# kendricktan/simple-zk-rollups

Measured on AMD Instinct MI355X. Metric: Groth16 proofs/sec (rollup batch circuit), higher is better.
Workload: dtype u32 limbs, 254-bit integer Montgomery (9 x 29 bits in the MSM kernels, 8 x 32 bits elsewhere); 1 GPU; 2^20-constraint synthetic rollup circuit, 1 proof per step per GPU; log_m=20, n_public=73, nVars=1048576, nnzA=1827887, nnzB=1577678, parallelism=proof-sharded x1 (key arena replicated once: single), proofs_in_flight=2

## Files before the change

### simple-zk-rollups_amd/csrc/curve29.hpp

```cpp
#pragma once
#include "curve.hpp"
#include "field29.hpp"

namespace zkr {

struct G1C {
  template <int H> using T = L29<Fq29, H>;
  using W = Fq;
  template <int H> static ZKR_HD T<H> unpack(const Fq &w) { return unpack29<Fq29, H>(w.v); }
  template <int H> static ZKR_HD Fq pack(const T<H> &a) { Fq r; pack29(a, r.v); return r; }
  static ZKR_HD T<2> one() { return one29<Fq29>(); }
  static ZKR_HD T<2> to256() { return const29<Fq29>(Fq29::TO256); }
  static ZKR_HD T<2> to261() { return const29<Fq29>(Fq29::TO261); }
};
struct G2C {
  template <int H> using T = Q29<H>;
  using W = Fq2;
  template <int H> static ZKR_HD T<H> unpack(const Fq2 &w) { return Q29<H>{unpack29<Fq29, H>(w.a.v), unpack29<Fq29, H>(w.b.v)}; }
  template <int H> static ZKR_HD Fq2 pack(const T<H> &x) { Fq2 r; pack29(x.a, r.a.v); pack29(x.b, r.b.v); return r; }
  static ZKR_HD T<2> one() { return Q29<2>{one29<Fq29>(), L29<Fq29, 2>::zero()}; }
  static ZKR_HD T<2> to256() { return Q29<2>{const29<Fq29>(Fq29::TO256), L29<Fq29, 2>::zero()}; }
  static ZKR_HD T<2> to261() { return Q29<2>{const29<Fq29>(Fq29::TO261), L29<Fq29, 2>::zero()}; }
};
template <class F> struct CoordOf;
template <> struct CoordOf<Fq> { using C = G1C; };
template <> struct CoordOf<Fq2> { using C = G2C; };

constexpr int HX = 13, HY = 4;

template <class C>
struct Affine29 {
  typename C::template T<2> x, y;
};
template <class C>
struct XYZZ29 {
  typename C::template T<HX> x;
  typename C::template T<HY> y, zz, zzz;
  static ZKR_HD XYZZ29 inf() {
    XYZZ29 r;
    r.x = decltype(r.x)::zero(); r.y = decltype(r.y)::zero(); r.zz = decltype(r.zz)::zero(); r.zzz = decltype(r.zzz)::zero();
    return r;
  }
  ZKR_HD bool is_inf() const { return zz.all_zero(); }
};
template <class C, class X, class Y, class ZZ, class ZZZ>
ZKR_HD XYZZ29<C> make_xyzz(const X &x, const Y &y, const ZZ &zz, const ZZZ &zzz) {
  XYZZ29<C> r;
  r.x = x.template to<HX>(); r.y = y.template to<HY>(); r.zz = zz.template to<HY>(); r.zzz = zzz.template to<HY>();
  return r;
}

template <class F>
ZKR_HD Affine29<typename CoordOf<F>::C> unpack_affine(const Affine<F> &p) {
  using C = typename CoordOf<F>::C;
  return Affine29<C>{C::template unpack<2>(p.x), C::template unpack<2>(p.y)};
}
template <class F>
ZKR_HD XYZZ29<typename CoordOf<F>::C> unpack_xyzz(const XYZZ<F> &p) {
  using C = typename CoordOf<F>::C;
  XYZZ29<C> r;
  r.x = C::template unpack<HY>(p.x).template to<HX>();
  r.y = C::template unpack<HY>(p.y); r.zz = C::template unpack<HY>(p.zz); r.zzz = C::template unpack<HY>(p.zzz);
  return r;
}
template <class F>
ZKR_HD XYZZ<F> pack_xyzz(const XYZZ29<typename CoordOf<F>::C> &p) {
  using C = typename CoordOf<F>::C;
  if (p.is_inf()) return XYZZ<F>::inf();
  return XYZZ<F>{C::template pack<3>(weak(p.x)), C::template pack<HY>(p.y), C::template pack<HY>(p.zz), C::template pack<HY>(p.zzz)};
}

template <class C, class QX, class QY>
ZKR_HD XYZZ29<C> dbl_affine29(const QX &qx, const QY &qy) {
  auto u = dbl(qy);
  auto v = sqr(u);
  auto w = mul(u, v);
  auto s = mul(qx, v);
  auto xx = sqr(qx);
  auto m = add(dbl(xx), xx);
  auto x3 = sub(sqr(m), dbl(s));
  auto y3 = mul_sub(m, sub_factor(s, x3), w, qy);
  return make_xyzz<C>(x3, y3, v, w);
}

template <class C>
ZKR_HD XYZZ29<C> dbl_xyzz29(const XYZZ29<C> &p) {
  if (p.is_inf()) return p;
  auto u = dbl(p.y);
  auto v = sqr(u);
  auto w = mul(u, v);
  auto s = mul(p.x, v);
  auto xx = sqr(p.x);
  auto m = add(dbl(xx), xx);
  auto x3 = sub(sqr(m), dbl(s));
  auto y3 = mul_sub(m, sub_factor(s, x3), w, p.y);
  return make_xyzz<C>(x3, y3, mul(v, p.zz), mul(w, p.zzz));
}

#if defined(__HIP_DEVICE_COMPILE__)
#define ZKR_PIN_ORDER() __builtin_amdgcn_sched_barrier(0)
#else
#define ZKR_PIN_ORDER() ((void)0)
#endif
template <class C>
ZKR_HD XYZZ29<C> add_mixed29(const XYZZ29<C> &acc, const Affine29<C> &q, bool neg_q) {
  if (acc.is_inf()) {
    auto qy = q.y;
    if (neg_q) qy = neg(q.y).template to<2>();
    return make_xyzz<C>(q.x, qy, C::one(), C::one());
  }
  auto u2 = mul(q.x, acc.zz);
  ZKR_PIN_ORDER();
  auto s2 = mul_cneg(q.y, neg_q, acc.zzz);
  ZKR_PIN_ORDER();
  auto p = sub(u2, acc.x);
  auto r = sub(s2, acc.y);
  auto pp = sqr(p);
  if (maybe_zero_mod_p(pp) && is_zero_mod_p(pp)) {
    if (is_zero_mod_p(sqr(r))) {
      auto qy = q.y;
      if (neg_q) qy = neg(q.y).template to<2>();
      return dbl_affine29<C>(q.x, qy);
    }
    return XYZZ29<C>::inf();
  }
  ZKR_PIN_ORDER();
  auto ppp = mul(p, pp);
  ZKR_PIN_ORDER();
  auto qq = mul(acc.x, pp);
  ZKR_PIN_ORDER();
  auto zz3 = mul(acc.zz, pp);
  ZKR_PIN_ORDER();
  auto zzz3 = mul(acc.zzz, ppp);
  ZKR_PIN_ORDER();
  auto x3 = sub_sub_dbl(sqr(r), ppp, qq);
  auto y3 = mul_sub(r, sub_factor(qq, x3), acc.y, ppp);
  return make_xyzz<C>(x3, y3, zz3, zzz3);
}

template <class C, class Again>
ZKR_HD XYZZ29<C> add_full29(const XYZZ29<C> &a, const XYZZ29<C> &b, Again again) {
  if (a.is_inf()) return b;
  if (b.is_inf()) return a;
  auto u1 = mul(a.x, b.zz);
  ZKR_PIN_ORDER();
  auto u2 = mul(b.x, a.zz);
  ZKR_PIN_ORDER();
  auto s1 = mul(a.y, b.zzz);
  ZKR_PIN_ORDER();
  auto s2 = mul(b.y, a.zzz);
  ZKR_PIN_ORDER();
  auto zzp = mul(a.zz, b.zz);
  ZKR_PIN_ORDER();
  auto zzzp = mul(a.zzz, b.zzz);
  ZKR_PIN_ORDER();
  auto p = sub(u2, u1);
  auto r = sub(s2, s1);
  auto pp = sqr(p);
  if (maybe_zero_mod_p(pp) && is_zero_mod_p(pp)) {
    if (is_zero_mod_p(sqr(r))) return dbl_xyzz29(again());
    return XYZZ29<C>::inf();
  }
  ZKR_PIN_ORDER();
  auto ppp = mul(p, pp);
  ZKR_PIN_ORDER();
  auto qq = mul(u1, pp);
  ZKR_PIN_ORDER();
  auto zz3 = mul(zzp, pp);
  ZKR_PIN_ORDER();
  auto zzz3 = mul(zzzp, ppp);
  ZKR_PIN_ORDER();
  auto x3 = sub_sub_dbl(sqr(r), ppp, qq);
  auto y3 = mul_sub(r, sub_factor(qq, x3), s1, ppp);
  return make_xyzz<C>(x3, y3, zz3, zzz3);
}
template <class C>
ZKR_HD XYZZ29<C> add_full29(const XYZZ29<C> &a, const XYZZ29<C> &b) {
  return add_full29<C>(a, b, [&]() { return b; });
}

constexpr int JX = 5, JY = 5, JZ = 8;
template <class C>
struct Jac29 {
  typename C::template T<JX> x;
  typename C::template T<JY> y;
  typename C::template T<JZ> z;
};
template <class C>
ZKR_HD Jac29<C> dbl_jac29(const Jac29<C> &p) {
  auto a = sqr(p.x);
  auto b = sqr(p.y);
  auto c8 = dbl(dbl(dbl(sqr(b))));
  auto s = dbl(dbl(mul(p.x, b)));
  auto e = add(dbl(a), a);
  auto x3 = barrett(sub(sqr(e), dbl(s)));
  auto y3 = barrett(sub(mul(e, sub(s, x3)), c8));
  auto z3 = dbl(mul(p.y, p.z));
  return Jac29<C>{x3.template to<JX>(), y3.template to<JY>(), z3.template to<JZ>()};
}

template <class F>
ZKR_HD_COLD F radix_to_261(const F &w) {
  using C = typename CoordOf<F>::C;
  return C::template pack<2>(canonical(mul(C::template unpack<10>(w), C::to261())));
}
template <class F>
ZKR_HD_COLD F radix_to_256(const F &w) {
  using C = typename CoordOf<F>::C;
  return C::template pack<2>(canonical(mul(C::template unpack<10>(w), C::to256())));
}
template <class F>
ZKR_HD_COLD void radix_to_261_at(F *w) {
  using C = typename CoordOf<F>::C;
  *w = C::template pack<2>(canonical_small(mul(C::template unpack<10>(*w), C::to261())));
}
template <class F>
ZKR_HD_COLD void radix_to_256_at(F *w) {
  using C = typename CoordOf<F>::C;
  *w = C::template pack<2>(canonical_small(mul(C::template unpack<10>(*w), C::to256())));
}
// ... 13 lines not shown
```

### simple-zk-rollups_amd/csrc/field29.hpp

```cpp
#pragma once
#include <utility>
#include "field.hpp"
#include "field29_consts.hpp"

namespace zkr {

constexpr uint32_t M29 = (1u << 29) - 1u;

template <class PM, int H>
struct L29 {
  static_assert(H >= 1 && H <= 128, "value bound out of range: the top limb has to stay below 2^28 (reductions take it as a signed word)");
  static constexpr int bound = H;
  uint32_t v[9];
  static ZKR_HD L29 zero() {
    L29 r;
#pragma unroll
    for (int i = 0; i < 9; i++) r.v[i] = 0;
    return r;
  }
  ZKR_HD bool all_zero() const {
    uint32_t o = 0;
#pragma unroll
    for (int i = 0; i < 9; i++) o |= v[i];
    return o == 0;
// ... 342 lines not shown
  int32_t c = 0;
#pragma unroll
  for (int i = 0; i < 9; i++) {
    t += (uint64_t)q * PM::P[i];
    const uint32_t ti = i < 8 ? (uint32_t)t & M29 : (uint32_t)t;
    t >>= 29;
    const int32_t d = (int32_t)a.v[i] - (int32_t)ti + c;
    if (i < 8) { r.v[i] = (uint32_t)d & M29; c = d >> 29; } else r.v[i] = (uint32_t)d;
  }
  return r;
}
template <class PM, int HA>
ZKR_HD L29<PM, 2> canonical_small(const L29<PM, HA> &a) {
  static_assert(HA <= 6, "reduce first (barrett / weak): one conditional subtraction per half-modulus pair");
  L29<PM, 2> r;
#pragma unroll
  for (int i = 0; i < 9; i++) r.v[i] = a.v[i];
#pragma unroll
  for (int it = 0; it < (HA - 1) / 2; it++) {
    int32_t c = 0;
    uint32_t d[9];
#pragma unroll
    for (int i = 0; i < 9; i++) {
      const int32_t t = (int32_t)r.v[i] - (int32_t)PM::P[i] + c;
      if (i < 8) { d[i] = (uint32_t)t & M29; c = t >> 29; } else { d[i] = (uint32_t)t; c = t >> 31; }
    }
    const bool ge = c == 0;
#pragma unroll
    for (int i = 0; i < 9; i++) r.v[i] = ge ? d[i] : r.v[i];
  }
  return r;
}

template <class PM, int HA>
ZKR_HD bool is_zero_mod_p(const L29<PM, HA> &a) {
  static_assert(HA <= 4, "reduce first: the test compares with 0 and p only");
  uint32_t z = 0, e = 0;
#pragma unroll
  for (int i = 0; i < 9; i++) { z |= a.v[i]; e |= a.v[i] ^ PM::P[i]; }
  return z == 0 || e == 0;
}
template <class PM, int HA>
ZKR_HD bool maybe_zero_mod_p(const L29<PM, HA> &a) {
  static_assert(HA <= 4, "reduce first: the test compares with 0 and p only");
  return a.v[0] == 0 || a.v[0] == PM::P[0];
}
template <class PM, int HA>
ZKR_HD_COLD L29<PM, 2> canonical(const L29<PM, HA> &a) {
  L29<PM, 2> r;
  uint32_t v[9];
#pragma unroll
  for (int i = 0; i < 9; i++) v[i] = a.v[i];
  for (int it = 0; it < (HA + 1) / 2; it++) {
    int32_t c = 0;
    uint32_t d[9];
    for (int i = 0; i < 9; i++) {
      int32_t t = (int32_t)v[i] - (int32_t)PM::P[i] + c;
      if (i < 8) { d[i] = (uint32_t)t & M29; c = t >> 29; } else { d[i] = (uint32_t)t; c = t >> 31; }
    }
    if (c == 0)
      for (int i = 0; i < 9; i++) v[i] = d[i];
  }
#pragma unroll
  for (int i = 0; i < 9; i++) r.v[i] = v[i];
  return r;
}

template <class PM29, class PM, int H = 2>
ZKR_HD L29<PM29, H> limbs_of(const Fp<PM> &a) {
  return unpack29<PM29, H>(a.v);
}
template <class PM, class PM29, int H>
ZKR_HD Fp<PM> words_of(const L29<PM29, H> &a) {
  Fp<PM> r;
  pack29(a, r.v);
  return r;
}

using Fq29 = Fq29Params;
using Fr29 = Fr29Params;

template <int H>
struct Q29 {
  L29<Fq29, H> a, b;
  static ZKR_HD Q29 zero() { return Q29{L29<Fq29, H>::zero(), L29<Fq29, H>::zero()}; }
  ZKR_HD bool all_zero() const { return a.all_zero() && b.all_zero(); }
  template <int H2>
  ZKR_HD Q29<H2> to() const { return Q29<H2>{a.template to<H2>(), b.template to<H2>()}; }
};
constexpr int neg_h(int h) { return 2 * ((h + 1) / 2); }
template <int HA, int HB>
ZKR_HD Q29<HA + HB> add(const Q29<HA> &x, const Q29<HB> &y) { return Q29<HA + HB>{add(x.a, y.a), add(x.b, y.b)}; }
template <int HA>
ZKR_HD Q29<2 * HA> dbl(const Q29<HA> &x) { return Q29<2 * HA>{dbl(x.a), dbl(x.b)}; }
template <int HA, int HB>
ZKR_HD Q29<HA + neg_h(HB)> sub(const Q29<HA> &x, const Q29<HB> &y) { return Q29<HA + neg_h(HB)>{sub(x.a, y.a), sub(x.b, y.b)}; }
template <int HB>
ZKR_HD Q29<neg_h(HB)> neg(const Q29<HB> &y) { return Q29<neg_h(HB)>{neg(y.a), neg(y.b)}; }
template <int HA, int HB, int HC>
ZKR_HD Q29<HA + 2 * ((HB + 2 * HC + 1) / 2)> sub_sub_dbl(const Q29<HA> &x, const Q29<HB> &y, const Q29<HC> &z) {
  return Q29<HA + 2 * ((HB + 2 * HC + 1) / 2)>{sub_sub_dbl(x.a, y.a, z.a), sub_sub_dbl(x.b, y.b, z.b)};
}
constexpr int max_h(int a, int b) { return a > b ? a : b; }
template <int HA, int HB>
ZKR_HD auto mul(const Q29<HA> &x, const Q29<HB> &y) {
  auto re = mul_sum2(x.a, y.a, neg_loose(x.b), y.b);
  auto im = mul_sum2(x.a, y.b, x.b, y.a);
  constexpr int H = max_h(decltype(re)::bound, decltype(im)::bound);
  return Q29<H>{re.template to<H>(), im.template to<H>()};
}
template <int HA>
ZKR_HD auto sqr(const Q29<HA> &x) {
  auto re = mul_sum2(x.a, x.a, neg_loose(x.b), x.b);
  auto im = mul(dbl(x.a), x.b);
  constexpr int H = max_h(decltype(re)::bound, decltype(im)::bound);
  return Q29<H>{re.template to<H>(), im.template to<H>()};
}
template <int HX, int HY, int HZ, int HW>
ZKR_HD auto mul_sub(const Q29<HX> &x, const Q29<HY> &y, const Q29<HZ> &z, const Q29<HW> &w) {
  auto nza = neg_loose(z.a);
  auto re = mul_sum4(x.a, y.a, neg_loose(x.b), y.b, nza, w.a, z.b, w.b);
  auto im = mul_sum4(x.a, y.b, x.b, y.a, nza, w.b, neg_loose(z.b), w.a);
  constexpr int H = max_h(decltype(re)::bound, decltype(im)::bound);
  return Q29<H>{re.template to<H>(), im.template to<H>()};
}
template <int HY, int HZ>
ZKR_HD auto mul_cneg(const Q29<HY> &y, bool flip, const Q29<HZ> &z) {
  auto pa = neg_loose(y.a), pb = neg_loose(y.b), nb = pb;
#pragma unroll
  for (int i = 0; i < 9; i++) {
    const uint32_t na = pa.v[i], nbi = pb.v[i];
    pa.v[i] = flip ? na : y.a.v[i];
    pb.v[i] = flip ? nbi : y.b.v[i];
    nb.v[i] = flip ? y.b.v[i] : nbi;
  }
  auto re = mul_sum2(z.a, pa, z.b, nb);
  auto im = mul_sum2(z.b, pa, z.a, pb);
  constexpr int H = max_h(decltype(re)::bound, decltype(im)::bound);
  return Q29<H>{re.template to<H>(), im.template to<H>()};
}
template <int HA, int HB>
ZKR_HD auto sub_factor(const Q29<HA> &x, const Q29<HB> &y) { return sub(x, y); }
template <int HA>
ZKR_HD Q29<3> weak(const Q29<HA> &x) { return Q29<3>{weak(x.a), weak(x.b)}; }
template <int HA>
ZKR_HD bool is_zero_mod_p(const Q29<HA> &x) { return is_zero_mod_p(x.a) && is_zero_mod_p(x.b); }
template <int HA>
ZKR_HD bool maybe_zero_mod_p(const Q29<HA> &x) { return maybe_zero_mod_p(x.a); }
template <int HA>
ZKR_HD_COLD Q29<2> canonical(const Q29<HA> &x) { return Q29<2>{canonical(x.a), canonical(x.b)}; }

template <int HA>
ZKR_HD Q29<5> barrett(const Q29<HA> &x) { return Q29<5>{barrett(x.a), barrett(x.b)}; }
template <int HA>
ZKR_HD Q29<2> canonical_small(const Q29<HA> &x) { return Q29<2>{canonical_small(x.a), canonical_small(x.b)}; }

template <class PM, int HA>
ZKR_HD L29<PM, 4> inv29(const L29<PM, HA> &a) {
  static_assert(HA * 4 <= 676, "operand bound too wide for the chain's products");
  static_assert(PM::P[0] >= 2, "p - 2 is taken limb-wise without a borrow");
  L29<PM, 4> r = one29<PM>().template to<4>();
#pragma unroll 1
  for (int i = 253; i >= 0; i--) {
    r = sqr(r).template to<4>();
    const uint32_t limb = PM::P[i / 29] - (i / 29 == 0 ? 2u : 0u);
    if ((limb >> (i % 29)) & 1u) r = mul(r, a).template to<4>();
  }
  return r;
}
template <int HA>
ZKR_HD Q29<4> inv29(const Q29<HA> &x) {
  auto ni = inv29(mul_sum2(x.a, x.a, x.b, x.b));
  return Q29<4>{mul(x.a, ni).template to<4>(), mul(neg(x.b), ni).template to<4>()};
}

}
```

### simple-zk-rollups_amd/csrc/host_arith_shim.cpp

```cpp
#include "hostops.hpp"
#include "pairing.hpp"
#include "curve29.hpp"
using namespace zkr;

namespace {
template <class P29> L29<P29, 3> to_m261(const uint8_t *std32) {
  uint32_t w[8];
  memcpy(w, std32, 32);
  return mul(unpack29<P29, 10>(w), const29<P29>(P29::R2)).template to<3>();
}
template <class P29, int H> void from_m261(const L29<P29, H> &x, uint8_t *std32) {
  L29<P29, 2> raw_one = L29<P29, 2>::zero();
  raw_one.v[0] = 1;
  uint32_t w[8];
  pack29(canonical(mul(x, raw_one)), w);
  memcpy(std32, w, 32);
}
template <class P29> void f29_op(int op, const uint8_t *a32, const uint8_t *b32, uint8_t *out) {
  auto a = to_m261<P29>(a32), b = to_m261<P29>(b32);
  switch (op) {
    case 0: from_m261(mul(a, b), out); break;
    case 1: from_m261(sqr(a), out); break;
    case 2: from_m261(add(a, b), out); break;
    case 3: from_m261(sub(a, b), out); break;
    case 4: from_m261(neg(a), out); break;
    case 5: from_m261(mul_sub(a, b, b, a), out); break;
    case 6: from_m261(mul_sum2(a, a, b, b), out); break;
    case 7: {
      auto t = sub(sub(a, b), sub(b, a));
      auto u = add(t, dbl(add(a, b)));
      from_m261(sqr(weak(u)), out);
      break;
    }
    case 8: from_m261(mul_sum4(a, b, a, a, b, b, neg(a), b), out); break;
    case 9: from_m261(weak(sub(sub(sub(a, b), b), b)), out); break;
    case 11: from_m261(mul(a, neg_loose(b)), out); break;
    case 12: from_m261(mul(b, sub_loose(a, b)), out); break;
    case 13: from_m261(mul_sum2(a, sub_loose(a, b), neg_loose(b), a), out); break;
    case 14: from_m261(mul_cneg(a, true, b), out); break;
    case 15: from_m261(mul_cneg(a, false, b), out); break;
    default: from_m261(mul(sub(a, b).template to<17>(), sub(b, a).template to<17>()), out);
  }
}
}

template <class F> static int chain29(const uint8_t *pts, const uint8_t *signs, size_t n, int twice, uint8_t *out) {
  using C = typename CoordOf<F>::C;
  const size_t pb = sizeof(Affine<F>);
  XYZZ29<C> half[2] = {XYZZ29<C>::inf(), XYZZ29<C>::inf()};
  for (size_t i = 0; i < n; i++) {
    Affine<F> p;
    memcpy(&p, pts + i * pb, pb);
    if (p.is_inf()) continue;
    Affine<F> q{radix_to_261(p.x), radix_to_261(p.y)};
    XYZZ29<C> &acc = half[i >= n / 2];
    acc = add_mixed29<C>(acc, unpack_affine(q), signs[i] != 0);
    acc = unpack_xyzz(pack_xyzz<F>(acc));
  }
  XYZZ29<C> tot = add_full29<C>(half[0], half[1]);
  if (twice) tot = add_full29<C>(tot, unpack_xyzz(pack_xyzz<F>(tot)));
  XYZZ<F> res = xyzz_to_256(pack_xyzz<F>(tot));
  if (res.is_inf()) return 1;
  Affine<F> a = to_affine(res);
  if constexpr (sizeof(F) == 32) store_g1_std(out, *reinterpret_cast<G1Affine *>(&a));
  else store_g2_std(out, *reinterpret_cast<G2Affine *>(&a));
  return 0;
}
template <class F> static void jac_levels29(const uint8_t *pt, int c, int levels, uint8_t *out) {
  using C = typename CoordOf<F>::C;
  Affine<F> p;
  memcpy(&p, pt, sizeof p);
  p.x = radix_to_261(p.x); p.y = radix_to_261(p.y);
  Jac29<C> q{C::template unpack<2>(p.x).template to<JX>(), C::template unpack<2>(p.y).template to<JY>(), C::one().template to<JZ>()};
  std::vector<Jac29<C>> lv;
  auto prod = C::one().template to<4>();
  for (int l = 0; l < levels; l++) {
    for (int b = 0; b < c; b++) q = dbl_jac29<C>(q);
    lv.push_back(q);
    prod = mul(prod, q.z).template to<4>();
  }
  auto inv = inv29(prod);
  for (int l = levels - 1; l >= 0; l--) {
    auto pre = C::one().template to<4>();
    for (int j = 0; j < l; j++) pre = mul(pre, lv[j].z).template to<4>();
    auto iz = mul(inv, pre);
    inv = mul(inv, lv[l].z).template to<4>();
    auto iz2 = sqr(iz);
    auto iz3 = mul(iz2, iz);
    Affine<F> a{radix_to_256(C::template pack<2>(canonical_small(mul(lv[l].x, iz2)))), radix_to_256(C::template pack<2>(canonical_small(mul(lv[l].y, iz3))))};
    if constexpr (sizeof(F) == 32) store_g1_std(out + (size_t)l * 64, *reinterpret_cast<G1Affine *>(&a));
    else store_g2_std(out + (size_t)l * 128, *reinterpret_cast<G2Affine *>(&a));
  }
}

#include <atomic>
#include <thread>
#include "shard_group.hpp"

static int shard_group_selftest(unsigned parts, unsigned rounds, unsigned fail_part, unsigned fail_round) {
  zkr::ShardGroup g;
  g.parts = parts;
  g.vecs.resize(parts);
  std::vector<std::atomic<unsigned>> at(parts);
  for (auto &a : at) a.store(0);
  std::atomic<int> bad{0};
  auto work = [&](unsigned i) {
    for (unsigned r = 0; r < rounds; r++) {
      if (i == fail_part && r == fail_round) { g.abort(); return; }
      at[i].store(r + 1);
      const bool ok = g.barrier();
      if (!ok) { if (fail_part >= parts || r < fail_round) bad++; return; }
      for (unsigned j = 0; j < parts; j++)
        if (at[j].load() < r + 1) bad++;
    }
    if (fail_part < parts && fail_round < rounds) bad++;
  };
  std::vector<std::thread> thr;
  for (unsigned i = 1; i < parts; i++) thr.emplace_back(work, i);
  work(0);
  for (auto &t : thr) t.join();
  return bad.load();
}

extern "C" {
int zkr_host_shard_group_selftest(unsigned parts, unsigned rounds, unsigned fail_part, unsigned fail_round) {
  return shard_group_selftest(parts, rounds, fail_part, fail_round);
}
void zkt29_fp(int field, int op, const uint8_t *a, const uint8_t *b, uint8_t *out) {
  if (field == 0) f29_op<Fq29>(op, a, b, out); else f29_op<Fr29>(op, a, b, out);
}
void zkt29_radix_roundtrip(const uint8_t *in32, uint8_t *out32, uint8_t *mid32) {
  Fq w;
  memcpy(w.v, in32, 32);
  Fq m = radix_to_261(w);
  memcpy(mid32, m.v, 32);
  Fq back = radix_to_256(m);
  memcpy(out32, back.v, 32);
}
void zkt29_raw_forms(int field, int form, const uint32_t *records, size_t n, uint32_t *out) {
  for (size_t i = 0; i < n; i++) {
    uint32_t op[8][9], r[9];
    memcpy(op, records + i * 72, sizeof op);
    if (field == 0) f29_raw_form<Fq29>(form, op, r); else f29_raw_form<Fr29>(form, op, r);
    memcpy(out + i * 9, r, sizeof r);
  }
}
void zkt29_barrett(int field, const uint32_t *in, uint32_t *out, uint32_t *canon) {
  if (field == 0) {
    L29<Fq29, 128> a; memcpy(a.v, in, 36);
    auto b = barrett(a); memcpy(out, b.v, 36);
    auto c = canonical_small(b); memcpy(canon, c.v, 36);
  } else {
    L29<Fr29, 128> a; memcpy(a.v, in, 36);
    auto b = barrett(a); memcpy(out, b.v, 36);
    auto c = canonical_small(b); memcpy(canon, c.v, 36);
  }
}
void zkt29_loose(int field, const uint32_t *a9, const uint32_t *b9, uint32_t *nl, uint32_t *sl, int *k_neg, int *k_sub) {
  if (field == 0) {
    L29<Fq29, 4> a; L29<Fq29, 13> b; memcpy(a.v, a9, 36); memcpy(b.v, b9, 36);
    auto n = neg_loose(b); auto d = sub_loose(a, b);
    memcpy(nl, n.v, 36); memcpy(sl, d.v, 36); *k_neg = decltype(n)::bound / 2; *k_sub = (decltype(d)::bound - 4) / 2;
  } else {
    L29<Fr29, 4> a; L29<Fr29, 13> b; memcpy(a.v, a9, 36); memcpy(b.v, b9, 36);
    auto n = neg_loose(b); auto d = sub_loose(a, b);
    memcpy(nl, n.v, 36); memcpy(sl, d.v, 36); *k_neg = decltype(n)::bound / 2; *k_sub = (decltype(d)::bound - 4) / 2;
  }
}
void zkt29_g1_levels(const uint8_t *pt, int c, int levels, uint8_t *out) { jac_levels29<Fq>(pt, c, levels, out); }
void zkt29_g2_levels(const uint8_t *pt, int c, int levels, uint8_t *out) { jac_levels29<Fq2>(pt, c, levels, out); }
int zkt29_g1_chain(const uint8_t *pts, const uint8_t *signs, size_t n, int twice, uint8_t *out) { return chain29<Fq>(pts, signs, n, twice, out); }
int zkt29_g2_chain(const uint8_t *pts, const uint8_t *signs, size_t n, int twice, uint8_t *out) { return chain29<Fq2>(pts, signs, n, twice, out); }

void zkt_fp(int field, int op, const uint8_t *a, const uint8_t *b, uint8_t *out) {
  if (field == 0) {
    Fq x = to_mont(load_fp<FqParams>(a)), y = to_mont(load_fp<FqParams>(b)), r;
    switch (op) { case 0: r = mul(x, y); break; case 1: r = add(x, y); break; case 2: r = sub(x, y); break;
                  case 3: r = inv(x); break; case 4: r = neg(x); break; default: r = sqr(x); }
    store_fp(out, from_mont(r));
  } else {
    Fr x = to_mont(load_fp<FrParams>(a)), y = to_mont(load_fp<FrParams>(b)), r;
    switch (op) { case 0: r = mul(x, y); break; case 1: r = add(x, y); break; case 2: r = sub(x, y); break;
                  case 3: r = inv(x); break; case 4: r = neg(x); break; default: r = sqr(x); }
    store_fp(out, from_mont(r));
  }
}
void zkt_fq2(int op, const uint8_t *a, const uint8_t *b, uint8_t *out) {
  Fq2 x{to_mont(load_fp<FqParams>(a)), to_mont(load_fp<FqParams>(a + 32))};
  Fq2 y{to_mont(load_fp<FqParams>(b)), to_mont(load_fp<FqParams>(b + 32))};
  Fq2 r = op == 0 ? mul(x, y) : op == 1 ? sqr(x) : inv(x);
  store_fp(out, from_mont(r.a));
  store_fp(out + 32, from_mont(r.b));
}
int zkt_g1_mul(const uint8_t *p_mont, const uint8_t *k32, uint8_t *out) {
  G1Affine p = load_g1(p_mont);
  U256 k = load_u256(k32);
  G1XYZZ acc = G1XYZZ::inf();
  for (int i = 255; i >= 0; i--) {
    acc = dbl_xyzz(acc);
    if ((k.v[i >> 5] >> (i & 31)) & 1) acc = add_mixed(acc, p);
  }
  if (acc.is_inf()) return 1;
  store_g1_std(out, to_affine(acc));
  return 0;
}
int zkt_g2_mul(const uint8_t *p_mont, const uint8_t *k32, uint8_t *out) {
  G2Affine p = load_g2(p_mont);
  U256 k = load_u256(k32);
  G2XYZZ acc = scalar_mul(to_xyzz(p), k);
  if (acc.is_inf()) return 1;
  store_g2_std(out, to_affine(acc));
  return 0;
}
int zkt_g1_lincomb(const uint8_t *p_mont, uint32_t a, uint32_t b, int negate_b, uint8_t *out) {
  G1Affine p = load_g1(p_mont);
  G1XYZZ pa = mul_small(to_xyzz(p), a), pb = mul_small(to_xyzz(p), b);
  G1XYZZ r;
  if (!pb.is_inf()) {
    G1Affine qb = to_affine(pb);
    r = add_mixed(pa, qb, negate_b != 0);
  } else {
    r = pa;
  }
  if (r.is_inf()) return 1;
  store_g1_std(out, to_affine(r));
  return 0;
}
int zkt_final_exp_check(uint64_t seed, int count) {
  using namespace zkr::pairing;
  uint64_t st = seed ? seed : 88172645463325252ull;
  auto rnd = [&]() { st ^= st << 13; st ^= st >> 7; st ^= st << 17; return (uint32_t)(st >> 16); };
  auto rfq = [&]() { Fq a; for (int i = 0; i < 8; i++) a.v[i] = rnd(); a.v[7] &= 0x0fffffffu; return to_mont(a); };
  auto rfq2 = [&]() { Fq2 r; r.a = rfq(); r.b = rfq(); return r; };
  auto rfq6 = [&]() { Fq6 r; r.c0 = rfq2(); r.c1 = rfq2(); r.c2 = rfq2(); return r; };
  uint32_t q[8];
  for (int i = 0; i < 8; i++) q[i] = FqParams::P[i];
  int ok = 0;
  for (int it = 0; it < count; it++) {
    Fq12 f{rfq6(), rfq6()};
    Fq12 fq = pow(f, q);
    ok += (fq == frobenius(f)) && (pow(fq, q) == frobenius2(f)) && (final_exponentiation_plain(f) == final_exponentiation(f));
  }
  return ok;
}
int zkt_miller_loops_agree(const uint8_t *g1, const uint8_t *g2, uint64_t seed, int count) {
  using namespace zkr::pairing;
  uint64_t st = seed ? seed : 88172645463325252ull;
  auto rnd = [&]() { st ^= st << 13; st ^= st >> 7; st ^= st << 17; return (uint32_t)(st >> 16); };
  G1Affine P{to_mont(load_fp<FqParams>(g1)), to_mont(load_fp<FqParams>(g1 + 32))};
  G2Affine Q{Fq2{to_mont(load_fp<FqParams>(g2)), to_mont(load_fp<FqParams>(g2 + 32))}, Fq2{to_mont(load_fp<FqParams>(g2 + 64)), to_mont(load_fp<FqParams>(g2 + 96))}};
  auto g2_mul = [&](uint32_t k) {
    G2XYZZ acc = G2XYZZ::inf();
    for (int b = 31; b >= 0; b--) { acc = dbl_xyzz(acc); if ((k >> b) & 1) acc = add_mixed(acc, Q); }
    return to_affine(acc);
  };
  int agree = 0;
// ... 44 lines not shown
```

### simple-zk-rollups_amd/csrc/kernels_msm.hpp

```cpp
#pragma once
#include "curve.hpp"
#include "curve29.hpp"

namespace zkr {

#define ZKR_RED_PRIO 3
constexpr int MSM_THREADS = 256;
constexpr uint32_t BIG_CAP = 1024;

template <class F> struct PointBytes;
template <> struct PointBytes<Fq> { static constexpr int N16 = 4; };
template <> struct PointBytes<Fq2> { static constexpr int N16 = 8; };

template <class T>
__device__ __forceinline__ T load_pod(const T *p) {
  static_assert(sizeof(T) % 16 == 0, "16-byte granules");
  T r;
  const uint4 *q = reinterpret_cast<const uint4 *>(p);
  uint4 *d = reinterpret_cast<uint4 *>(&r);
#pragma unroll
  for (unsigned i = 0; i < sizeof(T) / 16; i++) d[i] = q[i];
  return r;
}
template <class T>
// ... 357 lines not shown
    __syncthreads();
    part[threadIdx.x] += v;
    __syncthreads();
  }
  uint32_t run = block_sums[blockIdx.x] + part[threadIdx.x] - s;
#pragma unroll
  for (int k = 0; k < SCAN_PER_THREAD; k++) {
    if (base + k < nb) {
      offsets[base + k] = run;
      bool big = false;
      if (c[k] > big_thresh) {
        uint32_t slot = atomicAdd(big_count, 1u);
        if (slot < big_cap) { big_list[slot] = base + k; counts[base + k] = BIG_MARK; big = true; }
      }
      atomicAdd(&s_hist[big ? 0u : size_bin(c[k])], 1u);
      run += c[k];
    }
  }
  if (blockIdx.x == 0 && threadIdx.x == 0) offsets[nb] = *total;
  __syncthreads();
  for (uint32_t b = threadIdx.x; b < SIZE_BINS; b += SCAN_THREADS)
    if (s_hist[b]) atomicAdd(&size_hist[b], s_hist[b]);
}

static_assert(SIZE_BINS == 1024, "msm_hist_kernel clears 2 * 1024 words of size_hist");

static __global__ __launch_bounds__(SCAN_THREADS) void msm_order_kernel(const uint32_t *counts, uint32_t nb, const uint32_t *size_hist, uint32_t *taken, uint32_t *order) {
  __shared__ uint32_t s_start[SIZE_BINS];
  __shared__ uint32_t s_hist[SIZE_BINS];
  __shared__ uint32_t part[SCAN_THREADS];
  constexpr uint32_t PER = SIZE_BINS / SCAN_THREADS;
  const uint32_t t = threadIdx.x;
  uint32_t v[PER], sum = 0;
#pragma unroll
  for (uint32_t q = 0; q < PER; q++) { v[q] = size_hist[SIZE_BINS - 1 - (t * PER + q)]; sum += v[q]; }
  part[t] = sum;
  for (uint32_t b = t; b < SIZE_BINS; b += SCAN_THREADS) s_hist[b] = 0;
  __syncthreads();
  for (uint32_t off = 1; off < SCAN_THREADS; off <<= 1) {
    uint32_t u = t >= off ? part[t - off] : 0;
    __syncthreads();
    part[t] += u;
    __syncthreads();
  }
  uint32_t run = part[t] - sum;
#pragma unroll
  for (uint32_t q = 0; q < PER; q++) { s_start[SIZE_BINS - 1 - (t * PER + q)] = run; run += v[q]; }
  uint32_t base = blockIdx.x * SCAN_BLOCK + t * SCAN_PER_THREAD;
  uint32_t bin[SCAN_PER_THREAD], rank[SCAN_PER_THREAD];
#pragma unroll
  for (int k = 0; k < SCAN_PER_THREAD; k++) {
    if (base + k < nb) {
      uint32_t c = counts[base + k];
      bin[k] = c == BIG_MARK ? 0u : size_bin(c);
      rank[k] = atomicAdd(&s_hist[bin[k]], 1u);
    }
  }
  __syncthreads();
  for (uint32_t b = t; b < SIZE_BINS; b += SCAN_THREADS) {
    uint32_t h = s_hist[b];
    if (h) s_hist[b] = s_start[b] + atomicAdd(&taken[b], h);
  }
  __syncthreads();
#pragma unroll
  for (int k = 0; k < SCAN_PER_THREAD; k++)
    if (base + k < nb) order[s_hist[bin[k]] + rank[k]] = base + k;
}

constexpr int ACC_ONTO = 1, ACC_ZERO_BIG = 2;
constexpr int ACC_THREADS = 256;
template <class F, int MINW, bool AHEAD>
static __global__ __launch_bounds__(ACC_THREADS) __attribute__((amdgpu_waves_per_eu(MINW, MINW))) void msm_accum_kernel(const Affine<F> *points, const uint32_t *offsets, const uint32_t *entries,
                                                                     uint32_t nb, const uint32_t *counts, const uint32_t *order, XYZZ<F> *buckets, int onto) {
  using C = typename CoordOf<F>::C;
  const uint32_t t = blockIdx.x * ACC_THREADS + threadIdx.x;
  if (t >= nb) return;
  const uint32_t b = order[t];
  if (counts[b] == BIG_MARK) {
    if (onto & ACC_ZERO_BIG) store_pod(buckets + b, XYZZ<F>::inf());
    return;
  }
  uint32_t o0 = offsets[b], o1 = offsets[b + 1];
  XYZZ29<C> acc = (onto & ACC_ONTO) ? unpack_xyzz(load_pod(buckets + b)) : XYZZ29<C>::inf();
  if (o0 < o1) {
    const uint32_t last = o1 - 1;
    uint32_t e = entries[o0], e1 = entries[min(o0 + 1, last)];
    if (AHEAD) {
      Affine<F> p = load_pod(points + (e >> 1));
      for (uint32_t j = o0; j < o1; j++) {
        const uint32_t e2 = entries[min(j + 2, last)];
        const Affine<F> pn = load_pod(points + (e1 >> 1));
        if (!p.is_inf()) acc = add_mixed29<C>(acc, unpack_affine(p), (e & 1) != 0);
        e = e1; e1 = e2; p = pn;
      }
    } else {
      for (uint32_t j = o0; j < o1; j++) {
        const uint32_t e2 = entries[min(j + 2, last)];
        const Affine<F> p = load_pod(points + (e >> 1));
        if (!p.is_inf()) acc = add_mixed29<C>(acc, unpack_affine(p), (e & 1) != 0);
        e = e1; e1 = e2;
      }
    }
  }
  store_pod(buckets + b, pack_xyzz<F>(acc));
}

template <class T>
__device__ __forceinline__ T lane_xor_words(const T &v, int mask) {
  static_assert(sizeof(T) % 4 == 0, "made of 32-bit words");
  T r;
  const uint32_t *src = reinterpret_cast<const uint32_t *>(&v);
  uint32_t *dst = reinterpret_cast<uint32_t *>(&r);
#pragma unroll
  for (unsigned i = 0; i < sizeof(T) / 4; i++) dst[i] = (uint32_t)__shfl_xor((int)src[i], mask);
  return r;
}
template <class F, int MINW, int SPLIT>
static __global__ __launch_bounds__(ACC_THREADS) __attribute__((amdgpu_waves_per_eu(MINW, MINW))) void msm_accum_split_kernel(const Affine<F> *points, const uint32_t *offsets, const uint32_t *entries,
                                                                     uint32_t nb, const uint32_t *counts, const uint32_t *order, XYZZ<F> *buckets, int onto) {
  const uint32_t t = blockIdx.x * ACC_THREADS + threadIdx.x;
  const uint32_t slot = t / SPLIT, sub = t % SPLIT;
  if (slot >= nb) return;
  const uint32_t b = order[slot];
  if (counts[b] == BIG_MARK) {
    if ((onto & ACC_ZERO_BIG) && sub == 0) store_pod(buckets + b, XYZZ<F>::inf());
    return;
  }
  using C = typename CoordOf<F>::C;
  const uint32_t o0 = offsets[b], o1 = offsets[b + 1];
  XYZZ29<C> acc = (onto & ACC_ONTO) && sub == 0 ? unpack_xyzz(load_pod(buckets + b)) : XYZZ29<C>::inf();
  uint32_t e = o0 + sub < o1 ? entries[o0 + sub] : 0u;
  for (uint32_t j = o0 + sub; j < o1; j += SPLIT) {
    uint32_t en = j + SPLIT < o1 ? entries[j + SPLIT] : 0u;
    Affine<F> p = load_pod(points + (e >> 1));
    if (!p.is_inf()) acc = add_mixed29<C>(acc, unpack_affine(p), (e & 1) != 0);
    e = en;
  }
  for (int m = 1; m < SPLIT; m <<= 1) acc = add_full29<C>(acc, lane_xor_words(acc, m));
  if (sub == 0) store_pod(buckets + b, pack_xyzz<F>(acc));
}

template <class F>
__device__ __forceinline__ XYZZ<F> tree_add(const XYZZ<F> &a, const XYZZ<F> &b) {
  using C = typename CoordOf<F>::C;
  return pack_xyzz<F>(add_full29<C>(unpack_xyzz(a), unpack_xyzz(b), [&]() { return unpack_xyzz(b); }));
}
constexpr int BIG_SPLIT = 8;
constexpr int BIG_SLOTS = 64;

template <class F>
__device__ __forceinline__ void msm_big_body(const Affine<F> *points, const uint32_t *offsets, const uint32_t *entries,
                                             const uint32_t *big_list, const uint32_t *big_count, uint32_t big_cap, XYZZ<F> *partials) {
  __builtin_amdgcn_s_setprio(ZKR_RED_PRIO);
  using C = typename CoordOf<F>::C;
  extern __shared__ __attribute__((aligned(16))) unsigned char smem[];
  XYZZ<F> *sh = reinterpret_cast<XYZZ<F> *>(smem);
  uint32_t nbig = min(*big_count, big_cap);
  uint32_t sub = blockIdx.x % BIG_SPLIT;
  for (uint32_t w = blockIdx.x / BIG_SPLIT; w < nbig; w += BIG_SLOTS) {
    uint32_t b = big_list[w];
    uint32_t o0 = offsets[b], o1 = offsets[b + 1];
    XYZZ29<C> acc = XYZZ29<C>::inf();
    for (uint32_t j = o0 + sub * MSM_THREADS + threadIdx.x; j < o1; j += MSM_THREADS * BIG_SPLIT) {
      uint32_t e = entries[j];
      Affine<F> p = load_pod(points + (e >> 1));
      if (!p.is_inf()) acc = add_mixed29<C>(acc, unpack_affine(p), (e & 1) != 0);
    }
    sh[threadIdx.x] = pack_xyzz<F>(acc);
    __syncthreads();
    for (uint32_t s = MSM_THREADS / 2; s > 0; s >>= 1) {
      if (threadIdx.x < s) sh[threadIdx.x] = tree_add(sh[threadIdx.x], sh[threadIdx.x + s]);
      __syncthreads();
    }
    if (threadIdx.x == 0) copy_pod(partials + (size_t)w * BIG_SPLIT + sub, sh);
    __syncthreads();
  }
}

template <class F>
__device__ __forceinline__ void msm_big_finish_body(const XYZZ<F> *partials, const uint32_t *big_list, const uint32_t *big_count,
                                                    uint32_t big_cap, XYZZ<F> *buckets, int onto) {
  __builtin_amdgcn_s_setprio(ZKR_RED_PRIO);
  uint32_t w = blockIdx.x * blockDim.x + threadIdx.x;
  if (w >= min(*big_count, big_cap)) return;
  using C = typename CoordOf<F>::C;
  XYZZ29<C> acc = unpack_xyzz(load_pod(partials + (size_t)w * BIG_SPLIT));
  for (int k = 1; k < BIG_SPLIT; k++) {
    const XYZZ<F> *src = partials + (size_t)w * BIG_SPLIT + k;
    acc = add_full29<C>(acc, unpack_xyzz(load_pod(src)), [&]() { return unpack_xyzz(load_pod(src)); });
  }
  if (onto) {
    const XYZZ<F> *src = buckets + big_list[w];
    acc = add_full29<C>(acc, unpack_xyzz(load_pod(src)), [&]() { return unpack_xyzz(load_pod(src)); });
  }
  store_pod(buckets + big_list[w], pack_xyzz<F>(acc));
}

template <class F>
__device__ __forceinline__ void msm_reduce1_body(const XYZZ<F> *buckets, MsmGeom g, XYZZ<F> *group_out) {
  __builtin_amdgcn_s_setprio(ZKR_RED_PRIO);
  uint32_t t = blockIdx.x * blockDim.x + threadIdx.x;
  const uint32_t ng = (g.nbw >> g.glog) * g.batch, gs = 1u << g.glog;
  if (t >= ng) return;
  using C = typename CoordOf<F>::C;
  const XYZZ<F> *B = buckets + (size_t)t * gs;
  XYZZ29<C> run = unpack_xyzz(load_pod(B + gs - 1)), T = run;
  for (int j = (int)gs - 2; j >= 0; j--) {
    run = add_full29<C>(run, unpack_xyzz(load_pod(B + j)), [&]() { return unpack_xyzz(load_pod(B + j)); });
    T = add_full29<C>(T, run, [&]() { return run; });
  }
  store_pod(group_out + t, pack_xyzz<F>(run));
  store_pod(group_out + (size_t)ng + t, pack_xyzz<F>(T));
}

template <class F>
__device__ __forceinline__ void msm_reduce2_body(const XYZZ<F> *group_out, MsmGeom g, XYZZ<F> *task_out) {
  __builtin_amdgcn_s_setprio(ZKR_RED_PRIO);
  extern __shared__ __attribute__((aligned(16))) unsigned char smem[];
  XYZZ<F> *sh = reinterpret_cast<XYZZ<F> *>(smem);
  const uint32_t nglog = (uint32_t)(g.c - 1 - g.glog), ng = 1u << nglog;
  const uint32_t j = blockIdx.x / g.S, q = blockIdx.x % g.S;
  const uint32_t proof = blockIdx.y;
  using C = typename CoordOf<F>::C;
  const XYZZ<F> *R = group_out + (size_t)proof * ng;
  XYZZ29<C> acc = XYZZ29<C>::inf();
  if (j < nglog) {
    const uint32_t half = ng / 2, u0 = (uint32_t)((uint64_t)half * q / g.S), u1 = (uint32_t)((uint64_t)half * (q + 1) / g.S);
    for (uint32_t u = u0 + threadIdx.x; u < u1; u += MSM_THREADS) {
      uint32_t t = ((u >> j) << (j + 1)) | (1u << j) | (u & ((1u << j) - 1u));
      acc = add_full29<C>(acc, unpack_xyzz(load_pod(R + t)), [&]() { return unpack_xyzz(load_pod(R + t)); });
    }
  } else {
    const XYZZ<F> *T = group_out + (size_t)ng * g.batch + (size_t)proof * ng;
    const uint32_t h = j - nglog, lo = h * ng / 2, len = (h + 1) * ng / 2 - lo;
    const uint32_t t0 = lo + (uint32_t)((uint64_t)len * q / g.S), t1 = lo + (uint32_t)((uint64_t)len * (q + 1) / g.S);
    for (uint32_t t = t0 + threadIdx.x; t < t1; t += MSM_THREADS) acc = add_full29<C>(acc, unpack_xyzz(load_pod(T + t)), [&]() { return unpack_xyzz(load_pod(T + t)); });
  }
  sh[threadIdx.x] = pack_xyzz<F>(acc);
  __syncthreads();
  for (uint32_t s = MSM_THREADS / 2; s > 0; s >>= 1) {
    if (threadIdx.x < s) sh[threadIdx.x] = tree_add(sh[threadIdx.x], sh[threadIdx.x + s]);
    __syncthreads();
  }
  if (threadIdx.x == 0) copy_pod(task_out + (size_t)proof * gridDim.x + blockIdx.x, sh);
}

template <class F>
__device__ __forceinline__ void msm_reduce3_body(const XYZZ<F> *task_out, MsmGeom g, XYZZ<F> *result) {
  __builtin_amdgcn_s_setprio(ZKR_RED_PRIO);
// ... 180 lines not shown
```

Before: 152.1 proofs/s.

## Skip zz/zzz multiplies on second bucket add and use Karatsuba Fq2 squaring

Bucket accumulation now tracks whether the accumulator still holds a single affine point (zz=zzz=1). When it does, the mixed add skips four multiplications (u2, s2, zz3, zzz3). Fq2 squaring switches to the (a+b)(a-b) form when limb bounds allow, replacing a sum-of-products with a plain product. Host test shims are added for both. The cost is runtime branches inside the hot add, which can diverge per lane and raise register pressure, for a saving on only one add per bucket.

```diff
diff --git a/simple-zk-rollups_amd/csrc/curve29.hpp b/simple-zk-rollups_amd/csrc/curve29.hpp
--- a/simple-zk-rollups_amd/csrc/curve29.hpp
+++ b/simple-zk-rollups_amd/csrc/curve29.hpp
@@ -103,15 +103,24 @@
 #define ZKR_PIN_ORDER() ((void)0)
 #endif
 template <class C>
-ZKR_HD XYZZ29<C> add_mixed29(const XYZZ29<C> &acc, const Affine29<C> &q, bool neg_q) {
+ZKR_HD XYZZ29<C> add_mixed29(const XYZZ29<C> &acc, const Affine29<C> &q, bool neg_q, bool acc_affine = false) {
   if (acc.is_inf()) {
     auto qy = q.y;
     if (neg_q) qy = neg(q.y).template to<2>();
     return make_xyzz<C>(q.x, qy, C::one(), C::one());
   }
-  auto u2 = mul(q.x, acc.zz);
-  ZKR_PIN_ORDER();
-  auto s2 = mul_cneg(q.y, neg_q, acc.zzz);
+  constexpr int HU = max_h(decltype(mul(q.x, acc.zz))::bound, 2), HS = max_h(decltype(mul_cneg(q.y, neg_q, acc.zzz))::bound, 2);
+  typename C::template T<HU> u2;
+  if (acc_affine) u2 = q.x.template to<HU>();
+  else u2 = mul(q.x, acc.zz).template to<HU>();
+  ZKR_PIN_ORDER();
+  typename C::template T<HS> s2;
+  if (acc_affine) {
+    s2 = q.y.template to<HS>();
+    if (neg_q) s2 = neg(q.y).template to<HS>();
+  } else {
+    s2 = mul_cneg(q.y, neg_q, acc.zzz).template to<HS>();
+  }
   ZKR_PIN_ORDER();
   auto p = sub(u2, acc.x);
   auto r = sub(s2, acc.y);
@@ -129,13 +138,30 @@
   ZKR_PIN_ORDER();
   auto qq = mul(acc.x, pp);
   ZKR_PIN_ORDER();
-  auto zz3 = mul(acc.zz, pp);
-  ZKR_PIN_ORDER();
-  auto zzz3 = mul(acc.zzz, ppp);
+  constexpr int HZZ = max_h(decltype(mul(acc.zz, pp))::bound, decltype(pp)::bound), HZZZ = max_h(decltype(mul(acc.zzz, ppp))::bound, decltype(ppp)::bound);
+  typename C::template T<HZZ> zz3;
+  if (acc_affine) zz3 = pp.template to<HZZ>();
+  else zz3 = mul(acc.zz, pp).template to<HZZ>();
+  ZKR_PIN_ORDER();
+  typename C::template T<HZZZ> zzz3;
+  if (acc_affine) zzz3 = ppp.template to<HZZZ>();
+  else zzz3 = mul(acc.zzz, ppp).template to<HZZZ>();
   ZKR_PIN_ORDER();
   auto x3 = sub_sub_dbl(sqr(r), ppp, qq);
   auto y3 = mul_sub(r, sub_factor(qq, x3), acc.y, ppp);
   return make_xyzz<C>(x3, y3, zz3, zzz3);
+}
+
+template <class C>
+ZKR_HD XYZZ29<C> add_affine29(const Affine29<C> &a, bool neg_a, const Affine29<C> &q, bool neg_q) {
+  return add_mixed29<C>(add_mixed29<C>(XYZZ29<C>::inf(), a, neg_a), q, neg_q, true);
+}
+
+template <class C>
+ZKR_HD void chain_add29(XYZZ29<C> &acc, bool &one_point, const Affine29<C> &q, bool neg_q) {
+  const bool starts = acc.is_inf();
+  acc = add_mixed29<C>(acc, q, neg_q, one_point);
+  one_point = starts;
 }
 
 template <class C, class Again>
diff --git a/simple-zk-rollups_amd/csrc/field29.hpp b/simple-zk-rollups_amd/csrc/field29.hpp
--- a/simple-zk-rollups_amd/csrc/field29.hpp
+++ b/simple-zk-rollups_amd/csrc/field29.hpp
@@ -448,6 +448,7 @@
 
 template <int H>
 struct Q29 {
+  static constexpr int bound = H;
   L29<Fq29, H> a, b;
   static ZKR_HD Q29 zero() { return Q29{L29<Fq29, H>::zero(), L29<Fq29, H>::zero()}; }
   ZKR_HD bool all_zero() const { return a.all_zero() && b.all_zero(); }
@@ -476,11 +477,23 @@
   return Q29<H>{re.template to<H>(), im.template to<H>()};
 }
 template <int HA>
-ZKR_HD auto sqr(const Q29<HA> &x) {
+ZKR_HD auto sqr_sum2(const Q29<HA> &x) {
   auto re = mul_sum2(x.a, x.a, neg_loose(x.b), x.b);
   auto im = mul(dbl(x.a), x.b);
   constexpr int H = max_h(decltype(re)::bound, decltype(im)::bound);
   return Q29<H>{re.template to<H>(), im.template to<H>()};
+}
+constexpr bool sqr2_fits(int h) { return 2 * h * (h + 2 * ((h + 1) / 2 + 1)) <= 676; }
+template <int HA>
+ZKR_HD auto sqr(const Q29<HA> &x) {
+  if constexpr (sqr2_fits(HA)) {
+    auto im = mul(dbl(x.a), x.b);
+    auto re = mul(add(x.a, x.b), sub_loose(x.a, x.b));
+    constexpr int H = max_h(decltype(re)::bound, decltype(im)::bound);
+    return Q29<H>{re.template to<H>(), im.template to<H>()};
+  } else {
+    return sqr_sum2(x);
+  }
 }
 template <int HX, int HY, int HZ, int HW>
 ZKR_HD auto mul_sub(const Q29<HX> &x, const Q29<HY> &y, const Q29<HZ> &z, const Q29<HW> &w) {
diff --git a/simple-zk-rollups_amd/csrc/host_arith_shim.cpp b/simple-zk-rollups_amd/csrc/host_arith_shim.cpp
--- a/simple-zk-rollups_amd/csrc/host_arith_shim.cpp
+++ b/simple-zk-rollups_amd/csrc/host_arith_shim.cpp
@@ -66,6 +66,58 @@
   else store_g2_std(out, *reinterpret_cast<G2Affine *>(&a));
   return 0;
 }
+template <class F> static int add_affine_host(const uint8_t *a_wire, int neg_a, const uint8_t *q_wire, int neg_q, int mode, uint8_t *out) {
+  using C = typename CoordOf<F>::C;
+  Affine<F> pa, pq;
+  memcpy(&pa, a_wire, sizeof pa);
+  memcpy(&pq, q_wire, sizeof pq);
+  const Affine29<C> a = unpack_affine(Affine<F>{radix_to_261(pa.x), radix_to_261(pa.y)}), q = unpack_affine(Affine<F>{radix_to_261(pq.x), radix_to_261(pq.y)});
+  XYZZ29<C> tot;
+  if (mode == 0) {
+    tot = add_affine29<C>(a, neg_a != 0, q, neg_q != 0);
+  } else if (mode == 1) {
+    auto ay = a.y;
+    if (neg_a) ay = neg(a.y).template to<2>();
+    tot = add_mixed29<C>(make_xyzz<C>(a.x, ay, C::one(), C::one()), q, neg_q != 0);
+  } else {
+    tot = XYZZ29<C>::inf();
+    bool one_point = false;
+    chain_add29<C>(tot, one_point, a, neg_a != 0);
+    chain_add29<C>(tot, one_point, q, neg_q != 0);
+  }
+  XYZZ<F> res = xyzz_to_256(pack_xyzz<F>(tot));
+  if (res.is_inf()) return 1;
+  Affine<F> r = to_affine(res);
+  if constexpr (sizeof(F) == 32) store_g1_std(out, *reinterpret_cast<G1Affine *>(&r));
+  else store_g2_std(out, *reinterpret_cast<G2Affine *>(&r));
+  return 0;
+}
+template <class F> static int chain_start29(const uint8_t *pts, const uint8_t *signs, size_t n, uint8_t *out) {
+  using C = typename CoordOf<F>::C;
+  XYZZ29<C> acc = XYZZ29<C>::inf();
+  bool one_point = false;
+  for (size_t i = 0; i < n; i++) {
+    Affine<F> p;
+    memcpy(&p, pts + i * sizeof p, sizeof p);
+    if (p.is_inf()) continue;
+    chain_add29<C>(acc, one_point, unpack_affine(Affine<F>{radix_to_261(p.x), radix_to_261(p.y)}), signs[i] != 0);
+  }
+  XYZZ<F> res = xyzz_to_256(pack_xyzz<F>(acc));
+  if (res.is_inf()) return 1;
+  Affine<F> r = to_affine(res);
+  if constexpr (sizeof(F) == 32) store_g1_std(out, *reinterpret_cast<G1Affine *>(&r));
+  else store_g2_std(out, *reinterpret_cast<G2Affine *>(&r));
+  return 0;
+}
+template <int H> static int fq2_sqr_raw_h(const uint32_t *a9, const uint32_t *b9, int form, uint32_t *re, uint32_t *im) {
+  Q29<H> x;
+  memcpy(x.a.v, a9, 36);
+  memcpy(x.b.v, b9, 36);
+  if (form == 0) { auto r = sqr(x); memcpy(re, r.a.v, 36); memcpy(im, r.b.v, 36); }
+  else { auto r = sqr_sum2(x); memcpy(re, r.a.v, 36); memcpy(im, r.b.v, 36); }
+  return sqr2_fits(H) ? 1 : 0;
+}
+
 template <class F> static void jac_levels29(const uint8_t *pt, int c, int levels, uint8_t *out) {
   using C = typename CoordOf<F>::C;
   Affine<F> p;
@@ -172,6 +224,20 @@
 int zkt29_g1_chain(const uint8_t *pts, const uint8_t *signs, size_t n, int twice, uint8_t *out) { return chain29<Fq>(pts, signs, n, twice, out); }
 int zkt29_g2_chain(const uint8_t *pts, const uint8_t *signs, size_t n, int twice, uint8_t *out) { return chain29<Fq2>(pts, signs, n, twice, out); }
 
+int zkt29_g1_add_affine(const uint8_t *a, int neg_a, const uint8_t *q, int neg_q, int mode, uint8_t *out) { return add_affine_host<Fq>(a, neg_a, q, neg_q, mode, out); }
+int zkt29_g2_add_affine(const uint8_t *a, int neg_a, const uint8_t *q, int neg_q, int mode, uint8_t *out) { return add_affine_host<Fq2>(a, neg_a, q, neg_q, mode, out); }
+int zkt29_g1_chain_start(const uint8_t *pts, const uint8_t *signs, size_t n, uint8_t *out) { return chain_start29<Fq>(pts, signs, n, out); }
+int zkt29_g2_chain_start(const uint8_t *pts, const uint8_t *signs, size_t n, uint8_t *out) { return chain_start29<Fq2>(pts, signs, n, out); }
+int zkt29_fq2_sqr_raw(int h, const uint32_t *a9, const uint32_t *b9, int form, uint32_t *re, uint32_t *im) {
+  switch (h) {
+    case 4: return fq2_sqr_raw_h<4>(a9, b9, form, re, im);
+    case 8: return fq2_sqr_raw_h<8>(a9, b9, form, re, im);
+    case 12: return fq2_sqr_raw_h<12>(a9, b9, form, re, im);
+    case 13: return fq2_sqr_raw_h<13>(a9, b9, form, re, im);
+    case 17: return fq2_sqr_raw_h<17>(a9, b9, form, re, im);
+    default: return -1;
+  }
+}
 void zkt_fp(int field, int op, const uint8_t *a, const uint8_t *b, uint8_t *out) {
   if (field == 0) {
     Fq x = to_mont(load_fp<FqParams>(a)), y = to_mont(load_fp<FqParams>(b)), r;
diff --git a/simple-zk-rollups_amd/csrc/kernels_msm.hpp b/simple-zk-rollups_amd/csrc/kernels_msm.hpp
--- a/simple-zk-rollups_amd/csrc/kernels_msm.hpp
+++ b/simple-zk-rollups_amd/csrc/kernels_msm.hpp
@@ -463,6 +463,7 @@
   }
   uint32_t o0 = offsets[b], o1 = offsets[b + 1];
   XYZZ29<C> acc = (onto & ACC_ONTO) ? unpack_xyzz(load_pod(buckets + b)) : XYZZ29<C>::inf();
+  bool one_point = false;
   if (o0 < o1) {
     const uint32_t last = o1 - 1;
     uint32_t e = entries[o0], e1 = entries[min(o0 + 1, last)];
@@ -471,14 +472,14 @@
       for (uint32_t j = o0; j < o1; j++) {
         const uint32_t e2 = entries[min(j + 2, last)];
         const Affine<F> pn = load_pod(points + (e1 >> 1));
-        if (!p.is_inf()) acc = add_mixed29<C>(acc, unpack_affine(p), (e & 1) != 0);
+        if (!p.is_inf()) chain_add29<C>(acc, one_point, unpack_affine(p), (e & 1) != 0);
         e = e1; e1 = e2; p = pn;
       }
     } else {
       for (uint32_t j = o0; j < o1; j++) {
         const uint32_t e2 = entries[min(j + 2, last)];
         const Affine<F> p = load_pod(points + (e >> 1));
-        if (!p.is_inf()) acc = add_mixed29<C>(acc, unpack_affine(p), (e & 1) != 0);
+        if (!p.is_inf()) chain_add29<C>(acc, one_point, unpack_affine(p), (e & 1) != 0);
         e = e1; e1 = e2;
       }
     }
@@ -510,11 +511,12 @@
   using C = typename CoordOf<F>::C;
   const uint32_t o0 = offsets[b], o1 = offsets[b + 1];
   XYZZ29<C> acc = (onto & ACC_ONTO) && sub == 0 ? unpack_xyzz(load_pod(buckets + b)) : XYZZ29<C>::inf();
+  bool one_point = false;
   uint32_t e = o0 + sub < o1 ? entries[o0 + sub] : 0u;
   for (uint32_t j = o0 + sub; j < o1; j += SPLIT) {
     uint32_t en = j + SPLIT < o1 ? entries[j + SPLIT] : 0u;
     Affine<F> p = load_pod(points + (e >> 1));
-    if (!p.is_inf()) acc = add_mixed29<C>(acc, unpack_affine(p), (e & 1) != 0);
+    if (!p.is_inf()) chain_add29<C>(acc, one_point, unpack_affine(p), (e & 1) != 0);
     e = en;
   }
   for (int m = 1; m < SPLIT; m <<= 1) acc = add_full29<C>(acc, lane_xor_words(acc, m));
@@ -542,10 +544,11 @@
     uint32_t b = big_list[w];
     uint32_t o0 = offsets[b], o1 = offsets[b + 1];
     XYZZ29<C> acc = XYZZ29<C>::inf();
+    bool one_point = false;
     for (uint32_t j = o0 + sub * MSM_THREADS + threadIdx.x; j < o1; j += MSM_THREADS * BIG_SPLIT) {
       uint32_t e = entries[j];
       Affine<F> p = load_pod(points + (e >> 1));
-      if (!p.is_inf()) acc = add_mixed29<C>(acc, unpack_affine(p), (e & 1) != 0);
+      if (!p.is_inf()) chain_add29<C>(acc, one_point, unpack_affine(p), (e & 1) != 0);
     }
     sh[threadIdx.x] = pack_xyzz<F>(acc);
     __syncthreads();
```

Result: no change. 152.9 proofs/s, median of 2 (+0.6%).
